# mdolab/adflow

Measured on AMD Instinct MI355X. Metric: Mcells*residual-evals/s, higher is better.
Workload: dtype f64

## Files before the change

### adflow_amd/csrc/api.hip

```cpp
#include <hip/hip_runtime.h>

#include <algorithm>
#include <cmath>
#include <cstdarg>
#include <cstdio>
#include <cstring>
#include <functional>
#include <map>
#include <string>
#include <tuple>
#include <vector>

#include "internal.h"
#include "flow_plan.h"

extern int g_march_kch, g_viscous_tiled, g_inviscid_march, g_roe_march, g_sa_march;
int g_test_fault = 0;
int g_rvec_joint = 1;
int g_pc_fused = 1;
int g_xcd_tiles = 2;

namespace {

std::string g_err;
int g_device = -1;
hipStream_t g_stream = nullptr;
hipStream_t g_streamB = nullptr, g_streamC = nullptr;
hipEvent_t g_evFork = nullptr, g_evB = nullptr, g_evC = nullptr, g_evB1 = nullptr;
hipStream_t g_streamX = nullptr;
hipEvent_t g_evPack = nullptr, g_evComm = nullptr;
int g_overlap = 1;
adflow_opts g_opts;
bool g_have_opts = false;
hipEvent_t g_events[64];
bool g_events_ready = false;
bool g_async = false;

int fail(const char* fmt, ...)
{
    char buf[1024];
    va_list ap;
    va_start(ap, fmt);
    vsnprintf(buf, sizeof buf, fmt, ap);
    va_end(ap);
    g_err = buf;
    return 1;
}

#define HIPCHK(expr)                                                                        \
    do {                                                                                    \
        hipError_t e_ = (expr);                                                             \
        if (e_ != hipSuccess) return fail("%s failed: %s (%s:%d)", #expr, hipGetErrorString(e_), __FILE__, __LINE__); \
    } while (0)

struct DevArr {
    double* base = nullptr;
    int ncomp = 0;
};

struct Block {
    adflow_block_desc d;
    BlkView v;
    long boxsize = 0;
    std::vector<void*> allocs;
// ... 862 lines not shown
        const double* own = which == ADFLOW_ARR_X ? b->d.x : which == ADFLOW_ARR_SI ? b->d.sI : which == ADFLOW_ARR_SJ ? b->d.sJ : b->d.sK;
        const unsigned bit = which == ADFLOW_ARR_X ? 1u : which == ADFLOW_ARR_SI ? 2u : which == ADFLOW_ARR_SJ ? 4u : 8u;
        if (host == own) b->geom_is_host |= bit; else b->geom_is_host &= ~bit;
        b->normals_from_x_ok = b->geom_is_host == 15 && normals_match_nodes(b);
    }
    return sync_and_check();
}

int adflow_gpu_time_step(int level, int onlyRadii)
{
    if (need_ready()) return 1;
    KParams kp = make_kparams(level, 1.0, 0);
    kp.onlyRadii = onlyRadii;
    if (time_step_level(level, kp)) return 1;
    return sync_and_check();
}

int adflow_gpu_initres(int level, int varStart, int varEnd)
{
    if (need_ready()) return 1;
    if (varEnd < varStart) return 0;
    KParams kp = make_kparams(level, 1.0, 0);
    int rc = for_level(level, [&](Block* b) {
        if (varStart < 1 || varEnd > b->v.nw) return fail("initres: variable range %d..%d outside 1..%d", varStart, varEnd, b->v.nw);
        return 0;
    });
    if (rc) return rc;
    LevelTab t;
    if (level_tab(level, &t)) return 1;
    launch_initres_level(t.tab, t.n, t.nx, t.ny, t.nz, kp, varStart - 1, varEnd - 1, g_stream);
    return sync_and_check();
}

static int enqueue_flow_fluxes(int level, const KParams& kp, const struct FlowPlan& P, bool needGrad);
static int source_terms_enqueue(int withBlank);

static int wall_stress_enqueue(int level, const KParams& kp, bool formGrad);

static bool has_wall_subfaces(int level);

static bool level_at_rest(int level)
{
    bool anyMoving = false;
    for_level(level, [&](Block* b) { anyMoving = anyMoving || b->v.sFace || b->v.moving; return 0; });
    return !anyMoving;
}

static void block_face_vectors(Block* b)
{
    if (b->face_vectors_valid) return;
    launch_face_vectors(b->v, g_stream);
    b->face_vectors_valid = true;
}
static int ensure_face_vectors(int level)
{
    return for_level(level, [&](Block* b) { block_face_vectors(b); return 0; });
}

static KParams res_kparams(int level, unsigned flags)
{
    KParams kp = make_kparams(level, 1.0, 0);
    kp.onlyRadii = !(flags & ADFLOW_RES_UPDATE_INTERMED);
    kp.coarseInit = 0;
    if (level == 1 && g_rvec_target) { kp.rvec = g_rvec_target; kp.rvecTurbScale = g_opts.turbResScale; }
    kp.dissApprox = (flags & ADFLOW_RES_DISS_APPROX) ? 1 : 0;
    if (kp.dissApprox && (flags & ADFLOW_RES_UPWIND_FIRST_ORDER)) kp.lumpedDiss = 1;
    return kp;
}

static FlowFacts flow_facts(int level, const KParams& kp, bool viscApprox, bool needGradHbm, bool dual = false,
                            unsigned resFlags = ADFLOW_RES_FLOW)
{
    FlowFacts f = {};
    f.spaceDiscr = kp.spaceDiscr; f.viscous = kp.viscous; f.fineGrid = kp.fineGrid; f.fwMode = kp.fwMode; f.dissApprox = kp.dissApprox;
    f.lumpedDiss = kp.lumpedDiss; f.limiter = kp.limiter; f.coarseInit = kp.coarseInit; f.onlyRadii = kp.onlyRadii;
    f.doScaling = kp.doScaling; f.rvec = kp.rvec != nullptr; f.rFil = kp.rFil; f.adis = kp.adis;
    f.viscApprox = viscApprox; f.needGradHbm = needGradHbm; f.dual = dual;
    f.wantFlow = (resFlags & ADFLOW_RES_FLOW) != 0; f.wantTurb = (resFlags & ADFLOW_RES_TURB) != 0;
    f.atRest = level_at_rest(level);
    f.rans = g_opts.equations == ADFLOW_RANS;
    f.eulerMarch = g_use_march; f.inviscidMarch = g_inviscid_march; f.roeMarch = g_roe_march; f.viscousTiled = g_viscous_tiled;
    f.saMarch = g_sa_march; f.pcFused = g_pc_fused; f.rvecJoint = g_rvec_joint; f.jacSnap = g_jac_snap;
    return f;
}

static int enqueue_flow_residual(int level, const KParams& kp, bool viscApprox = false, bool lowSpeed = true, bool stage0 = true,
                                 bool needGradHbm = false)
{
    const bool wallStress = stage0 && !viscApprox && kp.viscous && level == g_opts.groundLevel && fabs(kp.rFil) >= 1.e-10 &&
                            has_wall_subfaces(level);
    const FlowPlan P = plan_flow(flow_facts(level, kp, viscApprox, needGradHbm));
    if (enqueue_flow_fluxes(level, kp, P, needGradHbm)) return 1;
    if (wallStress)
        if (wall_stress_enqueue(level, kp, P.wallGradOnChip)) return 1;
    if (lowSpeed && level == 1 && source_terms_enqueue(1)) return 1;
    if (lowSpeed && g_opts.lowSpeedPreconditioner) {
        LevelTab t;
        if (level_tab(level, &t)) return 1;
        launch_low_speed_precond_level(t.tab, t.n, t.nx, t.ny, t.nz, kp, g_stream);
    }
    return 0;
}

static int enqueue_flow_fluxes(int level, const KParams& kp, const FlowPlan& P, bool needGrad)
{
    if (kp.spaceDiscr != ADFLOW_DISS_SCALAR && kp.spaceDiscr != ADFLOW_DISS_MATRIX && kp.spaceDiscr != ADFLOW_UPWIND)
        return fail("spaceDiscr=%d not supported (1 scalar, 2 matrix, 9 upwind)", kp.spaceDiscr);
    int nStale = 0, nBlk = 0;
    int rc = for_level(level, [&](Block* b) {
        if (!b->geom_uploaded) return fail("geometry of a level-%d block has not been uploaded", level);
        ++nBlk;
        if (P.needSensor && !b->ss_valid) ++nStale;
        return 0;
    });
    if (rc) return rc;
    if (nStale > 0) {
        if (nStale == nBlk) {
            LevelTab ts;
            if (level_tab(level, &ts)) return 1;
            launch_entropy_level(ts.tab, ts.n, ts.nx, ts.ny, ts.nz, g_stream);
        }
        for_level(level, [&](Block* b) {
            if (nStale != nBlk && !b->ss_valid) launch_entropy(b->v, g_stream);
            b->ss_valid = true;
            return 0;
        });
    }
    LevelTab t;
    if (level_tab(level, &t)) return 1;
    if ((P.needGfTiles && ensure_gf_tiles(level)) || (P.needTiles && ensure_tiles(level))) return 1;
    KParams kv = kp;
    kv.viscFirst = P.viscFirst ? 1 : 0;
    auto inviscid = [&]() -> int {
        switch (P.inviscid) {
        case InviscidK::EulerMarch: launch_euler_march(g_tab[level], g_tiles[level].first, g_tiles[level].second, kv, g_stream); return 0;
        case InviscidK::RoeMarch: return launch_roe_march(g_tab[level], g_tiles[level].first, g_tiles[level].second, kv, g_stream);
        case InviscidK::FaceMarch: return launch_inviscid_march(g_tab[level], g_tiles[level].first, g_tiles[level].second, kv, g_stream);
        case InviscidK::PcMarch: launch_pc_march(g_tab[level], g_tiles[level].first, g_tiles[level].second, kv, g_march_kch, g_stream); return 0;
        case InviscidK::LevelGather: launch_inviscid_level(t.tab, t.n, t.nx, t.ny, t.nz, kv, g_stream); return 0;
        case InviscidK::None: break;
        }
        return 0;
    };
    auto viscous = [&]() -> int {
        switch (P.viscous) {
        case ViscousK::GfMarch: launch_visc_gf(g_tab[level], g_gf_tiles[level].first, g_gf_tiles[level].second, kv, needGrad, g_stream); return 0;
        case ViscousK::ThinLayerMarch: launch_visc_march_approx(g_tab[level], g_tiles[level].first, g_tiles[level].second, kv, g_stream); return 0;
        case ViscousK::GatherExact: return for_level(level, [&](Block* b) { block_face_vectors(b); launch_viscous(b->v, kv, g_stream); return 0; });
        case ViscousK::GatherApprox: return for_level(level, [&](Block* b) { block_face_vectors(b); launch_viscous_approx(b->v, kv, g_stream); return 0; });
        case ViscousK::None: break;
        }
        return 0;
    };
    if (P.inviscid == InviscidK::EulerMarch) return inviscid();
    if (P.inviscid == InviscidK::PcMarch) {
        if (ensure_face_vectors(level)) return 1;
        phase_mark(4);
        if (inviscid()) return 1;
        phase_mark(5);
        return 0;
    }
    if (P.viscFirst) {
        if (ensure_face_vectors(level)) return 1;
        phase_mark(4);
        if (viscous()) return 1;
        phase_mark(5);
        return inviscid();
    }
    if (inviscid()) return 1;
    phase_mark(4);
    if (P.needFaceVectors && ensure_face_vectors(level)) return 1;
    if (P.viscous == ViscousK::GfMarch) phase_mark(5);
    return viscous();
}

int adflow_gpu_residual(int level, int rkStage)
{
    if (need_ready()) return 1;
    double rFil = 1.0;
    int fwMode = 0;
    if (g_opts.smoother == ADFLOW_RUNGE_KUTTA) {
        if (rkStage < 0 || rkStage >= g_opts.nRKStages) return fail("rkStage=%d outside 0..%d", rkStage, g_opts.nRKStages - 1);
        rFil = g_opts.cdisRK[rkStage];
        fwMode = 1;
    }
    KParams kp = make_kparams(level, rFil, fwMode);
    int rc = enqueue_flow_residual(level, kp, false, true, rkStage == 0);
    if (rc) return rc;
    return sync_and_check();
}

static int block_res_enqueue(int level, unsigned flags);
static int apply_bc_enqueue(int level, int secondHalo);
static int apply_turb_bc_enqueue(int level, int secondHalo);
static int apply_turb_and_flow_bc_enqueue(int level, int secondHalo, bool turbBC);
static int turb_bc_treatment_enqueue(int level, const KParams& kp);
static int turb_bc_apply_enqueue(int level, const KParams& kp, int secondHalo);
static int bc_coarse_corrections_enqueue(int coarseLevel, double fact);
static void bc_plan_drop(int level);
static int halo_exchange_enqueue(int level, int varStart, int varEnd, int commPressure, int commVisc, int nLayers);
static int early_pressure_exchange_enqueue(int level);
static int halo_exchange_close(int level, int varStart, int varEnd, int commPressure, int nLayers);
static int comm_exchange_begin(CommPattern* cp, BlkView* tab, unsigned mask, int nvar, bool* remoteOut);
static int comm_exchange_end(CommPattern* cp, BlkView* tab, unsigned mask, bool remote);
static int block_res_split_enqueue(int level, unsigned flags, const KParams& kp, const FlowPlan& P, int lStart, int lEnd, int* taken,
                                   const std::function<int()>& frontBCs);

static int block_res_split_enqueue(int level, unsigned flags, const KParams& kp, const FlowPlan& P, int lStart, int lEnd, int* taken,
                                   const std::function<int()>& frontBCs)
{
    *taken = 0;
    if (!g_split_eval || !g_overlap || g_phase_base > 0 || kp.rvec) return 0;
    const unsigned need = ADFLOW_RES_FLOW | ADFLOW_RES_HALO;
    if ((flags & need) != need || (flags & (ADFLOW_RES_DISS_APPROX | ADFLOW_RES_VISC_APPROX | ADFLOW_RES_UPDATE_INTERMED))) return 0;
    if (P.viscous != ViscousK::GfMarch || !P.viscFirst || (P.inviscid != InviscidK::RoeMarch && P.inviscid != InviscidK::FaceMarch) ||
        P.turb == TurbK::LevelGather || P.needTimeStep || !kp.fineGrid) return 0;
    const bool rans = P.turb == TurbK::SaMarch;
    const bool wall = has_wall_subfaces(level) && level == g_opts.groundLevel;
    if (!g_act.empty()) return 0;
    CommPattern* cp;
    if (build_comm(level, 2, &cp)) return 1;
    const bool messages = !cp->sends.empty() || !cp->recvs.empty();
    if (g_split_eval < 2 && !messages) return 0;
    if (g_bc_callback) return 0;
    unsigned mask; int nvar;
    if (halo_mask(lStart, lEnd, 1, 1, &mask, &nvar)) return 1;
    if (nvar == 0) return 0;
    LevelTab t;
    if (level_tab(level, &t)) return 1;
    int rc = for_level(level, [&](Block* b) {
        if (!b->geom_uploaded) return fail("geometry of a level-%d block has not been uploaded", level);
        if (rans && b->v.nw < 6) return fail("RANS/SA needs nw = 6 (block has %d)", b->v.nw);
        block_face_vectors(b);
        return 0;
    });
    if (rc) return rc;
    if (ensure_tiles(level) || ensure_gf_tiles(level) || (rans && ensure_sa_tiles(level))) return 1;
    *taken = 1;
    KParams kv = kp;
    kv.viscFirst = 1;
    bool forked = false;
    auto run = [&]() -> int {
        HIPCHK(hipEventRecord(g_evFork, g_stream));
        HIPCHK(hipStreamWaitEvent(g_streamB, g_evFork, 0));
        forked = true;
        if (rans) launch_sa_march(t.tab, g_sa_tiles_int[level].first, g_sa_tiles_int[level].second, kp, g_streamB, false);
        launch_visc_gf(g_tab[level], g_gf_tiles_int[level].first, g_gf_tiles_int[level].second, kv, false, g_streamB);
        HIPCHK(hipEventRecord(g_evB1, g_streamB));
        if (frontBCs()) return 1;
        if (g_test_fault & 2) return fail("test_fault: the split evaluation fails behind its fork");
        bool remote = false;
        if (comm_exchange_begin(cp, g_tab[level], mask, nvar, &remote)) return 1;
        if (comm_exchange_end(cp, g_tab[level], mask, remote)) return 1;
        if (halo_exchange_close(level, lStart, lEnd, 1, 2)) return 1;
        HIPCHK(hipEventRecord(g_evC, g_stream));
        HIPCHK(hipStreamWaitEvent(g_streamB, g_evC, 0));
        if (rans) launch_sa_march(t.tab, g_sa_tiles_bnd[level].first, g_sa_tiles_bnd[level].second, kp, g_streamB, false);
        HIPCHK(hipEventRecord(g_evB, g_streamB));
        launch_visc_gf(g_tab[level], g_gf_tiles_bnd[level].first, g_gf_tiles_bnd[level].second, kv, false, g_stream);
        HIPCHK(hipStreamWaitEvent(g_stream, g_evB1, 0));
        if (P.inviscid == InviscidK::RoeMarch ? launch_roe_march(g_tab[level], g_tiles[level].first, g_tiles[level].second, kv, g_stream)
                                              : launch_inviscid_march(g_tab[level], g_tiles[level].first, g_tiles[level].second, kv, g_stream))
            return 1;
        HIPCHK(hipStreamWaitEvent(g_stream, g_evB, 0));
        forked = false;
        return 0;
    };
    if (run()) {
        if (forked && hipEventRecord(g_evB, g_streamB) == hipSuccess) (void)hipStreamWaitEvent(g_stream, g_evB, 0);
        return 1;
    }
    if (wall && wall_stress_enqueue(level, kp, true)) return 1;
    return 0;
}

static int block_res_enqueue(int level, unsigned flags)
{
    if (need_ready()) return 1;
    phase_mark(0);
    KParams kp = res_kparams(level, flags);
    const bool viscApprox = (flags & ADFLOW_RES_VISC_APPROX) != 0;
    const FlowPlan P = plan_flow(flow_facts(level, kp, viscApprox, (flags & ADFLOW_RES_UPDATE_INTERMED) != 0, false, flags));
    int rc = 0;
    bool etotInClosures = false;
    if (flags & ADFLOW_RES_CLOSURES) {
        LevelTab tc;
        if (level_tab(level, &tc)) return 1;
        etotInClosures = (flags & ADFLOW_RES_HALO) && (flags & ADFLOW_RES_FLOW) && g_comm.count(std::make_pair(level, 2)) > 0;
        if (etotInClosures) {
            if (!g_floor_flag_dev) HIPCHK(hipMalloc((void**)&g_floor_flag_dev, sizeof(int)));
            HIPCHK(hipMemsetAsync(g_floor_flag_dev, 0, sizeof(int), g_stream));
        }
        launch_closures_level(tc.tab, tc.n, tc.nx, tc.ny, tc.nz, kp, g_stream, etotInClosures ? g_floor_flag_dev : nullptr);
        rc = for_level(level, [&](Block* b) {
            b->ss_valid = false;
            b->etot_consistent = false;
            return 0;
        });
        if (rc) return rc;
    }
    if (flags & ADFLOW_RES_HALO) {
        auto frontBCs = [&]() -> int {
            if (apply_turb_and_flow_bc_enqueue(level, 1, (flags & ADFLOW_RES_TURB) != 0)) return 1;
            if (g_bc_callback) {
                HIPCHK(hipStreamSynchronize(g_stream));
                g_bc_callback(level, 1);
            }
            return 0;
        };
        int lStart = 1, lEnd = (g_opts.equations == ADFLOW_RANS) ? 6 : 5;
        if ((flags & ADFLOW_RES_FLOW) && !(flags & ADFLOW_RES_TURB)) lEnd = 5;
        if (!(flags & ADFLOW_RES_FLOW) && (flags & ADFLOW_RES_TURB)) lStart = 6;
        if (g_comm.count(std::make_pair(level, 2))) {
            int taken = 0;
            const int flagLevelWas = g_etot_flag_level;
            if (etotInClosures) g_etot_flag_level = level;
            rc = block_res_split_enqueue(level, flags, kp, P, lStart, lEnd, &taken, frontBCs);
            if (!rc && !taken) {
                rc = frontBCs();
                if (!rc) rc = halo_exchange_enqueue(level, lStart, lEnd, 1, 1, 2);
            }
            g_etot_flag_level = flagLevelWas;
            if (rc) return 1;
            if (taken) return 0;
        } else if (frontBCs()) return 1;
    }
    phase_mark(1);
    kp.radiiInMarch = P.radiiInMarch ? 1 : 0;
    if (P.needTimeStep) {
        rc = time_step_level(level, kp);
        if (rc) return rc;
    }
    phase_mark(2);
    if (P.turb != TurbK::None) {
        rc = for_level(level, [&](Block* b) {
            if (b->v.nw < 6) return fail("RANS/SA needs nw = 6 (block has %d)", b->v.nw);
            return 0;
        });
        if (rc) return rc;
        LevelTab t;
        if (level_tab(level, &t)) return 1;
        if (P.turb == TurbK::SaMarch) {
            if (ensure_sa_tiles(level)) return 1;
            if (P.roeWritesTurbRvec) kp.rvecTurbFromDw = 1;
            launch_sa_march(t.tab, g_sa_tiles[level].first, g_sa_tiles[level].second, kp, g_stream, false);
        } else launch_sa_residual_level(t.tab, t.n, t.nx, t.ny, t.nz, kp, g_stream);
    }
    phase_mark(3);
    if (flags & ADFLOW_RES_FLOW) {
        rc = enqueue_flow_residual(level, kp, viscApprox, false, true, (flags & ADFLOW_RES_UPDATE_INTERMED) != 0);
        if (rc) return rc;
    }
    phase_mark(6);
    if (level == 1 && source_terms_enqueue(0)) return 1;
    return 0;
}

int adflow_gpu_actuator_register(int nRegions, const adflow_actuator_region* regions)
// ... 1281 lines not shown
    launch_apply_all_bc(t.tab, pl->d_ent, pl->d_order, pl->flow, kp, secondHalo, g_opts.eulerWallBCTreatment,
                        g_opts.viscWallBCTreatment, g_opts.outflowTreatment, g_opts.hScalingInlet, g_stream);
    return for_level(level, [&](Block* b) {
        if (!b->bc.empty()) b->ss_valid = false;
        return 0;
    });
}

static int ad_apply_bc_enqueue(int level, const KParams& kp, bool turbBC)
{
    BcPlan* pl;
    if (bc_plan(level, &pl)) return 1;
    if (pl->nent == 0) return 0;
    if (pl->anyEulerWall && g_opts.eulerWallBCTreatment == ADFLOW_WALLBC_QUADRATIC)
        return fail("eulerWallBCTreatment=%d: bcEulerWall has no quadratic extrapolation", g_opts.eulerWallBCTreatment);
    LevelTab t;
    if (level_tab(level, &t)) return 1;
    if (turbBC) ad_launch_turb_bc(g_ad_tab, t.n, pl->maxFace, pl->d_ent, pl->d_order, pl->ordinal, kp, 1, g_stream);
    std::vector<BcPhase> flow;
    for (const BcPhase& ph : pl->flow)
        if (ph.kind != BCP_EXTRAP && ph.kind != BCP_SUPERSONIC_INFLOW) flow.push_back(ph);
    ad_launch_apply_all_bc(g_ad_tab, pl->d_ent, pl->d_order, flow, kp, 1, g_opts.eulerWallBCTreatment, g_opts.viscWallBCTreatment,
                           g_opts.outflowTreatment, g_opts.hScalingInlet, g_stream);
    return 0;
}

static bool has_wall_subfaces(int level)
{
    BcPlan* pl;
    if (bc_plan(level, &pl)) return false;
    return pl->wall.count > 0;
}

static int wall_stress_enqueue(int level, const KParams& kp, bool formGrad)
{
    BcPlan* pl;
    if (bc_plan(level, &pl)) return 1;
    if (pl->wall.count == 0) return 0;
    LevelTab t;
    if (level_tab(level, &t)) return 1;
    launch_wall_stress(t.tab, pl->d_ent, pl->d_order, pl->wall, kp, formGrad, g_stream);
    return 0;
}

int adflow_gpu_download_wall_stress(int nn, int level, int sps, int mm, double* tau, double* q)
{
    Block* b = find_block(nn, level, sps);
    if (!b) return fail("block (%d,%d,%d) not registered", nn, level, sps);
    if (mm < 1 || mm > b->nViscBocos || mm > (int)b->bc.size()) return fail("download_wall_stress: subface %d is not a viscous subface of block %d", mm, nn);
    const BcFaceDev& f = b->bc[mm - 1];
    int r[4];
    bc_owned_range(f.faceID, f.icBeg, f.icEnd, f.jcBeg, f.jcEnd, b->v.il, b->v.jl, b->v.kl, r);
    const long no = (long)std::max(0, r[1] - r[0] + 1) * std::max(0, r[3] - r[2] + 1);
    if (no == 0 || !f.tauq) return 0;
    HIPCHK(hipStreamSynchronize(g_stream));
    if (tau) HIPCHK(hipMemcpy(tau, f.tauq, sizeof(double) * 6 * no, hipMemcpyDeviceToHost));
    if (q) HIPCHK(hipMemcpy(q, f.tauq + 6 * no, sizeof(double) * 3 * no, hipMemcpyDeviceToHost));
    return 0;
}

static int bc_coarse_corrections_enqueue(int coarseLevel, double fact)
{
    BcPlan* pl;
    if (bc_plan(coarseLevel, &pl)) return 1;
    if (pl->nent == 0) return 0;
    LevelTab t;
    if (level_tab(coarseLevel, &t)) return 1;
    launch_bc_coarse_corrections(t.tab, pl->d_ent, pl->d_order, pl->ordinal, fact, g_stream);
    return 0;
}

int adflow_gpu_apply_all_bc(int level, int secondHalo)
{
    if (need_ready()) return 1;
// ... 553 lines not shown
        if (!kv.second.h_sendProc.empty() || !kv.second.h_recvProc.empty() || g_comm_self) return false;
    return true;
#endif
}
}

static int mg_cycle_enqueue(const int32_t* cycling, int nSteps);

int adflow_gpu_mg_cycle(const int32_t* cycling, int nSteps)
{
    if (need_ready()) return 1;
    if (!cycling || nSteps < 1) return fail("mg_cycle: empty cycling strategy");
#ifndef HOSTSIM
    if (mg_graph_eligible()) {
        const bool same = (g_mgg.gen == g_state_gen && (int)g_mgg.cyc.size() == nSteps && !memcmp(g_mgg.cyc.data(), cycling, sizeof(int32_t) * nSteps));
        if (!same) {
            mg_graph_drop();
            g_mgg.cyc.assign(cycling, cycling + nSteps);
            g_mgg.gen = g_state_gen;
        }
        if (g_mgg.exec && block_flags() == g_mgg.pre) {
            HIPCHK(hipGraphLaunch(g_mgg.exec, g_stream));
            set_block_flags(g_mgg.post);
            return sync_and_check();
        }
        if (g_mgg.exec) {
            g_mgg.seen = 0;
        } else if (g_mgg.seen >= 1) {
            HIPCHK(hipStreamSynchronize(g_stream));
            g_mgg.pre = block_flags();
            if (hipStreamBeginCapture(g_stream, hipStreamCaptureModeThreadLocal) == hipSuccess) {
                const bool was = g_async;
                g_async = true;
                const int rc = mg_cycle_enqueue(cycling, nSteps);
                g_async = was;
                hipGraph_t gr = nullptr;
                const hipError_t e1 = hipStreamEndCapture(g_stream, &gr);
                if (rc == 0 && e1 == hipSuccess && gr && !(g_test_fault & 1) && hipGraphInstantiate(&g_mgg.exec, gr, nullptr, nullptr, 0) == hipSuccess) {
                    g_mgg.graph = gr;
                    g_mgg.post = block_flags();
                    HIPCHK(hipGraphLaunch(g_mgg.exec, g_stream));
                    return sync_and_check();
                }
                if (gr) (void)hipGraphDestroy(gr);
                (void)hipGetLastError();
                g_mgg.exec = nullptr;
                g_mgg.failed = true;
                set_block_flags(g_mgg.pre);
            } else {
                (void)hipGetLastError();
                g_mgg.failed = true;
            }
        }
        ++g_mgg.seen;
    }
#endif
    const bool was_async = g_async;
    g_async = true;
    const int rc = mg_cycle_enqueue(cycling, nSteps);
    g_async = was_async;
    if (rc) return rc;
    return sync_and_check();
}

static int mg_cycle_enqueue(const int32_t* cycling, int nSteps)
{
    int level = g_opts.groundLevel;
// ... 536 lines not shown
        std::vector<int4> h((size_t)tt.second);
        if (tt.second > 0) HIPCHK(hipMemcpy(h.data(), tt.first, sizeof(int4) * h.size(), hipMemcpyDeviceToHost));
        for (const int4& t : h)
            if (t.x >= 0) out[1] += 4.0 * (t.w - t.z + 3);
    }
    for (auto& kv : g_blocks) {
        if (std::get<0>(kv.first) != level || std::get<1>(kv.first) != 1) continue;
        const BlkView& v = kv.second->v;
        int ntx, nty, ntz;
        euler_march_tiles(v, &ntx, &nty, &ntz);
        out[2] += 4.0 * ntx * nty * (v.nz + ntz);
    }
    return 0;
}

int adflow_gpu_sync(void)
{
    if (g_device < 0) return fail("adflow_gpu_init has not been called");
    HIPCHK(hipGetLastError());
    HIPCHK(hipStreamSynchronize(g_stream));
    return 0;
}

int adflow_gpu_set_tuning(const char* key, int value)
{
    ++g_state_gen;
    if (!key) return fail("null tuning key");
    if (!strcmp(key, "euler_march")) { g_use_march = (value != 0); return 0; }
    if (!strcmp(key, "viscous_tiled")) { g_viscous_tiled = value; return 0; }
    if (!strcmp(key, "inviscid_march")) { g_inviscid_march = value; return 0; }
    if (!strcmp(key, "roe_march")) { g_roe_march = value; return 0; }
    if (!strcmp(key, "sa_march")) { g_sa_march = value; return 0; }
    if (!strcmp(key, "overlap")) { g_overlap = value; return 0; }
    if (!strcmp(key, "max_grid_z")) { g_max_grid_z = (value > 0) ? value : 65535; return 0; }
    if (!strcmp(key, "metric_from_x")) { g_metric_from_x = value; return 0; }
    if (!strcmp(key, "xcd_tiles")) {
        g_xcd_tiles = value;
        if (g_stream) (void)hipStreamSynchronize(g_stream);
        mg_graph_drop();
        for (auto& kv : g_tiles) (void)hipFree(kv.second.first);
        g_tiles.clear();
        return 0;
    }
    if (!strcmp(key, "phase_events")) {
        if (value != 0 && (value < 8 || value > 56)) return fail("phase_events: first slot must be 8..56 (or 0 = off)");
        g_phase_base = value;
        return 0;
    }
    if (!strcmp(key, "march_kch")) {
        if (value < 4) return fail("march_kch must be >= 4");
        g_march_kch = value;
        if (g_stream) (void)hipStreamSynchronize(g_stream);
        mg_graph_drop();
        for (auto* mp : {&g_tiles, &g_gf_tiles, &g_gf_tiles_int, &g_gf_tiles_bnd, &g_sa_tiles, &g_sa_tiles_int, &g_sa_tiles_bnd}) {
            for (auto& kv : *mp) (void)hipFree(kv.second.first);
            mp->clear();
        }
        return 0;
    }
    if (!strcmp(key, "split_eval")) { g_split_eval = value; return 0; }
    if (!strcmp(key, "test_fault")) { g_test_fault = value; g_mgg.failed = false; mg_graph_drop(); return 0; }
    if (!strcmp(key, "ad_cache")) { g_ad_cache = value; if (!value) { if (g_stream) (void)hipStreamSynchronize(g_stream); ad_drop(); } return 0; }
    if (!strcmp(key, "rvec_joint")) { g_rvec_joint = value; return 0; }
    if (!strcmp(key, "jac_snap")) { g_jac_snap = value; return 0; }
    if (!strcmp(key, "pc_fused")) { g_pc_fused = value; mg_graph_drop(); return 0; }
    if (!strcmp(key, "mg_graph")) { g_mg_graph = value; g_mgg.failed = false; mg_graph_drop(); return 0; }
// ... 65 lines not shown
```

### adflow_amd/csrc/internal.h

```cpp
#pragma once
#include <hip/hip_runtime.h>
#include <stdint.h>
#include "../../include/adflow_gpu.h"

#define ADF_PAD0 14

#ifdef HOSTSIM
#define GPTR(T) T*
#else
#define GPTR(T) T __attribute__((address_space(1)))*
#endif

__device__ __forceinline__ double ldg(GPTR(const double) base, unsigned byteoff)
{
    return *(GPTR(const double))((GPTR(const char))base + byteoff);
}
__device__ __forceinline__ void stg(GPTR(double) base, unsigned byteoff, double v)
{
    *(GPTR(double))((GPTR(char))base + byteoff) = v;
}

#ifndef ADF_NR
#define ADF_NR 1
#endif
// ... 347 lines not shown
void launch_source_terms(const BlkView* tab, const int* blk, const long* off, int n, const double Ffact[3], double Qfact, int withBlank,
                         hipStream_t s);
void launch_low_speed_precond_level(const BlkView* tab, int nslots, int maxnx, int maxny, int maxnz, const KParams& kp, hipStream_t s);
void launch_stage_update_level(const BlkView* tab, int nslots, int maxnx, int maxny, int maxnz, const KParams& kp, double scale,
                               int fromWn, hipStream_t s);
void launch_res_averaging_level(const BlkView* tab, int nslots, int maxnx, int maxny, int maxnz, const KParams& kp, hipStream_t s,
                                double scaleDtl = 0.0);
void launch_dadi_level(const BlkView* tab, int nslots, int nx, int ny, int nz, const KParams& kp, hipStream_t s, bool withUpdate = false);
void launch_halo_copy(const BlkView* tab, const int* donorBlk, const long* donorOff, const int* haloBlk, const long* haloOff,
                      int n, unsigned mask, hipStream_t s);
void launch_periodic(const BlkView* tab, const int* blk, const long* off, int n, const double rotMatrix[9], const double rotCenter[3],
                     const double translation[3], int coor, hipStream_t s);
void launch_halo_pack(const BlkView* tab, const int* blk, const long* off, int n, unsigned mask, double* buf, hipStream_t s);
void launch_halo_unpack(const BlkView* tab, const int* blk, const long* off, int n, unsigned mask, const double* buf,
                        hipStream_t s);
int launch_inviscid_march(const BlkView* tab, const int4* tiles, int ntiles, const KParams& kp, hipStream_t s);
int inviscid_march_enabled();
int launch_roe_march(const BlkView* tab, const int4* tiles, int ntiles, const KParams& kp, hipStream_t s);
void launch_pc_march(const BlkView* tab, const int4* tiles, int ntiles, const KParams& kp, int kch, hipStream_t s);
bool roe_march_takes(int limiter);
void launch_euler_march(const BlkView* tab, const int4* tiles, int ntiles, const KParams& kp, hipStream_t s);
void euler_march_tiles(const BlkView& b, int* ntx, int* nty, int* ntz);
void launch_restrict_level(const BlkView* ctab, const BlkView* ftab, int nslots, int nx, int ny, int nz, const KParams& kp, hipStream_t s);
void launch_store_entry_state_level(const BlkView* ctab, int nslots, int nx, int ny, int nz, hipStream_t s);
void launch_forcing_level(const BlkView* ctab, int nslots, int nx, int ny, int nz, double fcoll, hipStream_t s);
void launch_corrections_level(const BlkView* ctab, int nslots, int nx, int ny, int nz, hipStream_t s);
void launch_prolong_update_level(const BlkView* ftab, const BlkView* ctab, int nslots, int nx, int ny, int nz, const KParams& kp,
                                 hipStream_t s);
void launch_set_w(const BlkView& b, const double* vec, double turbFloor, hipStream_t s);
void launch_get_r(const BlkView& b, double* vec, double turbScale, double* sums, hipStream_t s);
void launch_closures(const BlkView& b, const KParams& kp, hipStream_t s);
void launch_closures_level(const BlkView* tab, int nslots, int maxnx, int maxny, int maxnz, const KParams& kp, hipStream_t s,
                           int* floored = nullptr);
void launch_set_w_closures_level(const BlkView* tab, int nslots, int maxnx, int maxny, int maxnz, const double* vec, double turbFloor,
                                 const KParams& kp, int* floored, hipStream_t s);
void launch_set_w_level(const BlkView* tab, int nslots, int maxnx, int maxny, int maxnz, const double* vec, double turbFloor, hipStream_t s);
void launch_get_r_level(const BlkView* tab, int nslots, int maxnx, int maxny, int maxnz, double* vec, double turbScale, double* sums, hipStream_t s);
void launch_entropy_level(const BlkView* tab, int nslots, int maxnx, int maxny, int maxnz, hipStream_t s);
void launch_etot_owned_level(const BlkView* tab, int nslots, int maxnx, int maxny, int maxnz, double gammaConstant, hipStream_t s,
                             const int* onlyIf = nullptr);
void launch_initres_level(const BlkView* tab, int nslots, int maxnx, int maxny, int maxnz, const KParams& kp, int l0, int l1, hipStream_t s);
void launch_res_norms(const BlkView& b, int nvar, double* out, hipStream_t s);
#include <vector>
void launch_apply_all_bc(const BlkView* tab, const BcEntry* ent, const int* order, const std::vector<BcPhase>& flow,
                         const KParams& kp, int second, int eulerWallTreatment, int viscWallTreatment, int outflowTreatment, int hScalingInlet,
                         hipStream_t s);
void launch_turb_bc_treatment(const BlkView* tab, int nslots, long maxFace, const BcEntry* ent, const int* order,
                              const std::vector<BcPhase>& ordinal, const KParams& kp, hipStream_t s);
void launch_apply_turb_bc(const BlkView* tab, const BcEntry* ent, const int* order, const std::vector<BcPhase>& ordinal,
                          const KParams& kp, int second, hipStream_t s);
void launch_bc_coarse_corrections(const BlkView* tab, const BcEntry* ent, const int* order, const std::vector<BcPhase>& ordinal,
                                  double fact, hipStream_t s);
void launch_corner_row_halos_level(const BlkView* tab, int nslots, const KParams& kp, hipStream_t s);
void launch_volume_metric(const BlkView& b, int rightHanded, hipStream_t s);
void launch_boundary_normals(const BlkView& b, const BcFaceDev* faces, int nBocos, hipStream_t s);
void launch_wall_distance(const BlkView& b, const int* ind, const double* uv, const double* xSurf, hipStream_t s);

void ad_launch_from_real(const double* src, void* dst, long n, hipStream_t s);
void ad_launch_value(const void* src, double* dst, long n, int deriv, hipStream_t s);
void ad_launch_snap(const BlkView& b, const void* dwd, double* snap, const JacSpec& J, double turbResScale, hipStream_t s);
void ad_launch_closures_halo(const BlkView& adv, const KParams& kp, hipStream_t s);
void ad_launch_apply_all_bc(const BlkView* tab, const BcEntry* ent, const int* order, const std::vector<BcPhase>& flow, const KParams& kp,
                            int second, int eulerWallTreatment, int viscWallTreatment, int outflowTreatment, int hScalingInlet, hipStream_t s);
void ad_launch_turb_bc(const BlkView* tab, int nslots, long maxFace, const BcEntry* ent, const int* order, const std::vector<BcPhase>& ordinal,
                       const KParams& kp, int second, hipStream_t s);
void ad_launch_time_step_level(const BlkView* tab, int n, int nx, int ny, int nz, const KParams& kp, hipStream_t s);
// ... 15 lines not shown
```

### adflow_amd/csrc/kernels_nk.hip

```cpp
#include <algorithm>

#include "internal.h"

#define NK_BX 64
#define NK_BY 4

__device__ __forceinline__ void set_w_body(const BlkView& b, int kz, const double* __restrict__ vec, double turbFloor)
{
    const int i = blockIdx.x * NK_BX + threadIdx.x + 2;
    const int j = blockIdx.y * NK_BY + threadIdx.y + 2;
    const int k = kz + 2;
    if (i > b.il || j > b.jl || k > b.kl) return;
    const long c = b.idx(i, j, k);
    const long m = (((long)(k - 2) * b.ny + (j - 2)) * b.nx + (i - 2)) * b.nw;
    for (int l = 0; l < 5; ++l) b.w[c + l * b.nbox] = vec[m + l];
    if (b.nw > 5) b.w[c + 5 * b.nbox] = fmax(turbFloor, vec[m + 5]);
}

__global__ __launch_bounds__(NK_BX* NK_BY) void k_set_w(BlkView b, const double* __restrict__ vec, double turbFloor)
{
    set_w_body(b, (int)blockIdx.z, vec, turbFloor);
}

__global__ __launch_bounds__(NK_BX* NK_BY) void k_set_w_level(const BlkView* __restrict__ tab, int nzb, const double* __restrict__ vec,
// ... 88 lines not shown
    }
    if (kp.viscous) {
        const double muSuth = kp.muSuthDim / kp.muRef, TSuth = kp.TSuthDim / kp.TRef, SSuth = kp.SSuthDim / kp.TRef;
        const double T = p / (kp.RGas * rho);
        const double tt = T / TSuth;
        const double rlv = muSuth * ((TSuth + SSuth) / (T + SSuth)) * (tt * sqrt(tt));
        b.rlv[c] = rlv;
        if (kp.eddyModel && kp.updateEddy) {
            const double cv13 = kp.sa_cv1 * kp.sa_cv1 * kp.sa_cv1;
            const double rnuSA = b.w[c + 5 * nb] * rho;
            const double chi = rnuSA / rlv;
            const double chi3 = chi * chi * chi;
            b.rev[c] = chi3 / (chi3 + cv13) * rnuSA;
        }
    }
}

__global__ __launch_bounds__(NK_BX* NK_BY) void k_closures(BlkView b, KParams kp) { closures_body(b, (int)blockIdx.z, kp); }

__global__ __launch_bounds__(NK_BX* NK_BY) void k_set_w_closures_level(const BlkView* __restrict__ tab, int nzb, const double* __restrict__ vec,
                                                                       double turbFloor, KParams kp, int* __restrict__ floored)
{
    const BlkView& b = tab[blockIdx.z / nzb + 1];
    set_w_body(b, (int)(blockIdx.z % nzb), vec + b.vecOff, turbFloor);
    closures_body<true>(b, (int)(blockIdx.z % nzb), kp, floored);
}

template <bool ETOT>
__global__ __launch_bounds__(NK_BX* NK_BY) void k_closures_level(const BlkView* __restrict__ tab, int nzb, KParams kp, int* __restrict__ floored)
{
    closures_body<ETOT>(tab[blockIdx.z / nzb + 1], (int)(blockIdx.z % nzb), kp, floored);
}

static dim3 nk_grid(const BlkView& b) { return dim3((b.nx + NK_BX - 1) / NK_BX, (b.ny + NK_BY - 1) / NK_BY, b.nz); }
static dim3 nk_level_grid(int nslots, int maxnx, int maxny, int maxnz)
{
    return dim3((maxnx + NK_BX - 1) / NK_BX, (maxny + NK_BY - 1) / NK_BY, maxnz * nslots);
}

void launch_closures_level(const BlkView* tab, int nslots, int maxnx, int maxny, int maxnz, const KParams& kp, hipStream_t s, int* floored)
{
    LEVEL_SPLIT(nslots, maxnz + 4, launch_closures_level(tab + s0_, n_, maxnx, maxny, maxnz, kp, s, floored));
    if (nslots <= 0) return;
    if (floored)
        hipLaunchKernelGGL(k_closures_level<true>, nk_level_grid(nslots, maxnx, maxny, maxnz), dim3(NK_BX, NK_BY, 1), 0, s, tab, maxnz, kp, floored);
    else
        hipLaunchKernelGGL(k_closures_level<false>, nk_level_grid(nslots, maxnx, maxny, maxnz), dim3(NK_BX, NK_BY, 1), 0, s, tab, maxnz, kp,
                           (int*)nullptr);
}
void launch_set_w_closures_level(const BlkView* tab, int nslots, int maxnx, int maxny, int maxnz, const double* vec, double turbFloor,
                                 const KParams& kp, int* floored, hipStream_t s)
{
    LEVEL_SPLIT(nslots, maxnz + 4, launch_set_w_closures_level(tab + s0_, n_, maxnx, maxny, maxnz, vec, turbFloor, kp, floored, s));
    if (nslots <= 0) return;
    hipLaunchKernelGGL(k_set_w_closures_level, nk_level_grid(nslots, maxnx, maxny, maxnz), dim3(NK_BX, NK_BY, 1), 0, s, tab, maxnz, vec, turbFloor,
                       kp, floored);
}
void launch_set_w_level(const BlkView* tab, int nslots, int maxnx, int maxny, int maxnz, const double* vec, double turbFloor, hipStream_t s)
{
    LEVEL_SPLIT(nslots, maxnz + 4, launch_set_w_level(tab + s0_, n_, maxnx, maxny, maxnz, vec, turbFloor, s));
    if (nslots <= 0) return;
    hipLaunchKernelGGL(k_set_w_level, nk_level_grid(nslots, maxnx, maxny, maxnz), dim3(NK_BX, NK_BY, 1), 0, s, tab, maxnz, vec, turbFloor);
}
void launch_get_r_level(const BlkView* tab, int nslots, int maxnx, int maxny, int maxnz, double* vec, double turbScale, double* sums, hipStream_t s)
{
    LEVEL_SPLIT(nslots, maxnz + 4, launch_get_r_level(tab + s0_, n_, maxnx, maxny, maxnz, vec, turbScale, sums, s));
    if (nslots <= 0) return;
    hipLaunchKernelGGL(k_get_r_level, nk_level_grid(nslots, maxnx, maxny, maxnz), dim3(NK_BX, NK_BY, 1), 0, s, tab, maxnz, vec, turbScale, sums);
}

void launch_set_w(const BlkView& b, const double* vec, double turbFloor, hipStream_t s)
{
    hipLaunchKernelGGL(k_set_w, nk_grid(b), dim3(NK_BX, NK_BY, 1), 0, s, b, vec, turbFloor);
}

void launch_get_r(const BlkView& b, double* vec, double turbScale, double* sums, hipStream_t s)
{
    hipLaunchKernelGGL(k_get_r, nk_grid(b), dim3(NK_BX, NK_BY, 1), 0, s, b, vec, turbScale, sums);
}

void launch_closures(const BlkView& b, const KParams& kp, hipStream_t s)
{
// ... 3 lines not shown
```

Baseline: 4874.

## Split closures into shell and bulk, overlap bulk and wall stress on side stream

The closures kernel is split into a shell launch covering the outer two layers of each block and a bulk launch covering the interior. The shell runs first, so boundary conditions and halo exchange can start while the interior closures run on a second stream and join before the fluxes. The wall-stress kernel is likewise moved to the side stream after the viscous-first pass so it can overlap the inviscid fluxes. This adds launches, events and more complex indexing in exchange for hiding closure and wall-stress work behind the front BCs and comms. Side-stream use is turned off during graph capture and when callbacks are active.

```diff
diff --git a/adflow_amd/csrc/api.hip b/adflow_amd/csrc/api.hip
--- a/adflow_amd/csrc/api.hip
+++ b/adflow_amd/csrc/api.hip
@@ -30,6 +30,8 @@
 hipStream_t g_streamX = nullptr;
 hipEvent_t g_evPack = nullptr, g_evComm = nullptr;
 int g_overlap = 1;
+int g_closures_split = 1;
+bool g_capturing = false;
 adflow_opts g_opts;
 bool g_have_opts = false;
 hipEvent_t g_events[64];
@@ -958,10 +960,12 @@
     return sync_and_check();
 }
 
-static int enqueue_flow_fluxes(int level, const KParams& kp, const struct FlowPlan& P, bool needGrad);
+static int enqueue_flow_fluxes(int level, const KParams& kp, const struct FlowPlan& P, bool needGrad,
+                               const std::function<int()>* afterViscousFirst = nullptr);
 static int source_terms_enqueue(int withBlank);
 
-static int wall_stress_enqueue(int level, const KParams& kp, bool formGrad);
+static int wall_stress_enqueue(int level, const KParams& kp, bool formGrad, hipStream_t s = g_stream);
+static bool side_queue_usable() { return g_overlap && g_phase_base == 0 && !g_bc_callback && !g_capturing; }
 
 static bool has_wall_subfaces(int level);
 
@@ -1016,9 +1020,23 @@
     const bool wallStress = stage0 && !viscApprox && kp.viscous && level == g_opts.groundLevel && fabs(kp.rFil) >= 1.e-10 &&
                             has_wall_subfaces(level);
     const FlowPlan P = plan_flow(flow_facts(level, kp, viscApprox, needGradHbm));
-    if (enqueue_flow_fluxes(level, kp, P, needGradHbm)) return 1;
-    if (wallStress)
-        if (wall_stress_enqueue(level, kp, P.wallGradOnChip)) return 1;
+    const bool wallBeside = wallStress && P.viscFirst && side_queue_usable();
+    bool forkMarked = false;
+    const std::function<int()> markFork = [&]() -> int {
+        HIPCHK(hipEventRecord(g_evFork, g_stream));
+        forkMarked = true;
+        return 0;
+    };
+    if (enqueue_flow_fluxes(level, kp, P, needGradHbm, wallBeside ? &markFork : nullptr)) return 1;
+    if (wallStress) {
+        if (forkMarked) {
+            HIPCHK(hipStreamWaitEvent(g_streamB, g_evFork, 0));
+            const int rc = wall_stress_enqueue(level, kp, P.wallGradOnChip, g_streamB);
+            if (hipEventRecord(g_evB, g_streamB) != hipSuccess || hipStreamWaitEvent(g_stream, g_evB, 0) != hipSuccess)
+                return fail("the side queue of the wall stress could not be joined");
+            if (rc) return rc;
+        } else if (wall_stress_enqueue(level, kp, P.wallGradOnChip)) return 1;
+    }
     if (lowSpeed && level == 1 && source_terms_enqueue(1)) return 1;
     if (lowSpeed && g_opts.lowSpeedPreconditioner) {
         LevelTab t;
@@ -1028,7 +1046,7 @@
     return 0;
 }
 
-static int enqueue_flow_fluxes(int level, const KParams& kp, const FlowPlan& P, bool needGrad)
+static int enqueue_flow_fluxes(int level, const KParams& kp, const FlowPlan& P, bool needGrad, const std::function<int()>* afterViscousFirst)
 {
     if (kp.spaceDiscr != ADFLOW_DISS_SCALAR && kp.spaceDiscr != ADFLOW_DISS_MATRIX && kp.spaceDiscr != ADFLOW_UPWIND)
         return fail("spaceDiscr=%d not supported (1 scalar, 2 matrix, 9 upwind)", kp.spaceDiscr);
@@ -1091,6 +1109,7 @@
         phase_mark(4);
         if (viscous()) return 1;
         phase_mark(5);
+        if (afterViscousFirst && (*afterViscousFirst)()) return 1;
         return inviscid();
     }
     if (inviscid()) return 1;
@@ -1129,29 +1148,42 @@
 static int halo_exchange_close(int level, int varStart, int varEnd, int commPressure, int nLayers);
 static int comm_exchange_begin(CommPattern* cp, BlkView* tab, unsigned mask, int nvar, bool* remoteOut);
 static int comm_exchange_end(CommPattern* cp, BlkView* tab, unsigned mask, bool remote);
+static int comm_exchange_enqueue(CommPattern* cp, BlkView* tab, unsigned mask, int nvar);
 static int block_res_split_enqueue(int level, unsigned flags, const KParams& kp, const FlowPlan& P, int lStart, int lEnd, int* taken,
                                    const std::function<int()>& frontBCs);
+static bool split_eval_applies(int level, unsigned flags, const KParams& kp, const FlowPlan& P, int lStart, int lEnd, int* err);
+
+static bool split_eval_applies(int level, unsigned flags, const KParams& kp, const FlowPlan& P, int lStart, int lEnd, int* err)
+{
+    *err = 0;
+    if (!g_split_eval || !g_overlap || g_phase_base > 0 || kp.rvec) return false;
+    const unsigned need = ADFLOW_RES_FLOW | ADFLOW_RES_HALO;
+    if ((flags & need) != need || (flags & (ADFLOW_RES_DISS_APPROX | ADFLOW_RES_VISC_APPROX | ADFLOW_RES_UPDATE_INTERMED))) return false;
+    if (P.viscous != ViscousK::GfMarch || !P.viscFirst || (P.inviscid != InviscidK::RoeMarch && P.inviscid != InviscidK::FaceMarch) ||
+        P.turb == TurbK::LevelGather || P.needTimeStep || !kp.fineGrid) return false;
+    if (!g_act.empty()) return false;
+    CommPattern* cp;
+    if (build_comm(level, 2, &cp)) { *err = 1; return false; }
+    const bool messages = !cp->sends.empty() || !cp->recvs.empty();
+    if (g_split_eval < 2 && !messages) return false;
+    if (g_bc_callback) return false;
+    unsigned mask; int nvar;
+    if (halo_mask(lStart, lEnd, 1, 1, &mask, &nvar)) { *err = 1; return false; }
+    return nvar > 0;
+}
 
 static int block_res_split_enqueue(int level, unsigned flags, const KParams& kp, const FlowPlan& P, int lStart, int lEnd, int* taken,
                                    const std::function<int()>& frontBCs)
 {
     *taken = 0;
-    if (!g_split_eval || !g_overlap || g_phase_base > 0 || kp.rvec) return 0;
-    const unsigned need = ADFLOW_RES_FLOW | ADFLOW_RES_HALO;
-    if ((flags & need) != need || (flags & (ADFLOW_RES_DISS_APPROX | ADFLOW_RES_VISC_APPROX | ADFLOW_RES_UPDATE_INTERMED))) return 0;
-    if (P.viscous != ViscousK::GfMarch || !P.viscFirst || (P.inviscid != InviscidK::RoeMarch && P.inviscid != InviscidK::FaceMarch) ||
-        P.turb == TurbK::LevelGather || P.needTimeStep || !kp.fineGrid) return 0;
+    int err = 0;
+    if (!split_eval_applies(level, flags, kp, P, lStart, lEnd, &err)) return err;
     const bool rans = P.turb == TurbK::SaMarch;
     const bool wall = has_wall_subfaces(level) && level == g_opts.groundLevel;
-    if (!g_act.empty()) return 0;
     CommPattern* cp;
     if (build_comm(level, 2, &cp)) return 1;
-    const bool messages = !cp->sends.empty() || !cp->recvs.empty();
-    if (g_split_eval < 2 && !messages) return 0;
-    if (g_bc_callback) return 0;
     unsigned mask; int nvar;
     if (halo_mask(lStart, lEnd, 1, 1, &mask, &nvar)) return 1;
-    if (nvar == 0) return 0;
     LevelTab t;
     if (level_tab(level, &t)) return 1;
     int rc = for_level(level, [&](Block* b) {
@@ -1209,15 +1241,37 @@
     const FlowPlan P = plan_flow(flow_facts(level, kp, viscApprox, (flags & ADFLOW_RES_UPDATE_INTERMED) != 0, false, flags));
     int rc = 0;
     bool etotInClosures = false;
+    bool bulkPending = false;
+    LevelTab tc;
+    int lStart = 1, lEnd = (g_opts.equations == ADFLOW_RANS) ? 6 : 5;
+    if ((flags & ADFLOW_RES_FLOW) && !(flags & ADFLOW_RES_TURB)) lEnd = 5;
+    if (!(flags & ADFLOW_RES_FLOW) && (flags & ADFLOW_RES_TURB)) lStart = 6;
+    auto bulkClosures = [&](hipStream_t s) -> int {
+        if (!bulkPending) return 0;
+        bulkPending = false;
+        launch_closures_bulk_level(tc.tab, tc.n, tc.nx, tc.ny, tc.nz, kp, s, etotInClosures ? g_floor_flag_dev : nullptr);
+        return 0;
+    };
     if (flags & ADFLOW_RES_CLOSURES) {
-        LevelTab tc;
         if (level_tab(level, &tc)) return 1;
         etotInClosures = (flags & ADFLOW_RES_HALO) && (flags & ADFLOW_RES_FLOW) && g_comm.count(std::make_pair(level, 2)) > 0;
         if (etotInClosures) {
             if (!g_floor_flag_dev) HIPCHK(hipMalloc((void**)&g_floor_flag_dev, sizeof(int)));
             HIPCHK(hipMemsetAsync(g_floor_flag_dev, 0, sizeof(int), g_stream));
         }
-        launch_closures_level(tc.tab, tc.n, tc.nx, tc.ny, tc.nz, kp, g_stream, etotInClosures ? g_floor_flag_dev : nullptr);
+        int* const floorFlag = etotInClosures ? g_floor_flag_dev : nullptr;
+        int err = 0;
+        const bool splitEval = etotInClosures && split_eval_applies(level, flags, kp, P, lStart, lEnd, &err);
+        if (err) return 1;
+        if (g_closures_split >= 2) {
+            if (g_closures_split == 2) launch_closures_shell_level(tc.tab, tc.n, tc.nx, tc.ny, tc.nz, kp, g_stream, floorFlag);
+            else launch_closures_bulk_level(tc.tab, tc.n, tc.nx, tc.ny, tc.nz, kp, g_stream, floorFlag);
+        } else if (g_closures_split == 1 && (flags & ADFLOW_RES_HALO) && kp.fineGrid && !splitEval &&
+                   std::min(tc.nx, std::min(tc.ny, tc.nz)) > 2 * CLOSURE_SHELL) {
+            launch_closures_shell_level(tc.tab, tc.n, tc.nx, tc.ny, tc.nz, kp, g_stream, floorFlag);
+            bulkPending = true;
+        } else
+            launch_closures_level(tc.tab, tc.n, tc.nx, tc.ny, tc.nz, kp, g_stream, floorFlag);
         rc = for_level(level, [&](Block* b) {
             b->ss_valid = false;
             b->etot_consistent = false;
@@ -1234,22 +1288,48 @@
             }
             return 0;
         };
-        int lStart = 1, lEnd = (g_opts.equations == ADFLOW_RANS) ? 6 : 5;
-        if ((flags & ADFLOW_RES_FLOW) && !(flags & ADFLOW_RES_TURB)) lEnd = 5;
-        if (!(flags & ADFLOW_RES_FLOW) && (flags & ADFLOW_RES_TURB)) lStart = 6;
+        auto frontWithBulk = [&](bool exchange) -> int {
+            bool forked = false;
+            auto run = [&]() -> int {
+                if (bulkPending && side_queue_usable()) {
+                    HIPCHK(hipEventRecord(g_evFork, g_stream));
+                    HIPCHK(hipStreamWaitEvent(g_streamB, g_evFork, 0));
+                    forked = true;
+                    if (bulkClosures(g_streamB)) return 1;
+                    HIPCHK(hipEventRecord(g_evB, g_streamB));
+                }
+                if (frontBCs()) return 1;
+                if (g_test_fault & 4) return fail("test_fault: the boundary front fails behind its fork");
+                unsigned mask = 0; int nvar = 0;
+                if (exchange) {
+                    CommPattern* cp;
+                    if (build_comm(level, 2, &cp)) return 1;
+                    if (halo_mask(lStart, lEnd, 1, 1, &mask, &nvar)) return 1;
+                    if (nvar > 0 && comm_exchange_enqueue(cp, g_tab[level], mask, nvar)) return 1;
+                }
+                if (bulkClosures(g_stream)) return 1;
+                if (forked) {
+                    HIPCHK(hipStreamWaitEvent(g_stream, g_evB, 0));
+                    forked = false;
+                }
+                return (exchange && nvar > 0) ? halo_exchange_close(level, lStart, lEnd, 1, 2) : 0;
+            };
+            if (run()) {
+                if (forked && hipEventRecord(g_evB, g_streamB) == hipSuccess) (void)hipStreamWaitEvent(g_stream, g_evB, 0);
+                return 1;
+            }
+            return 0;
+        };
         if (g_comm.count(std::make_pair(level, 2))) {
             int taken = 0;
             const int flagLevelWas = g_etot_flag_level;
             if (etotInClosures) g_etot_flag_level = level;
             rc = block_res_split_enqueue(level, flags, kp, P, lStart, lEnd, &taken, frontBCs);
-            if (!rc && !taken) {
-                rc = frontBCs();
-                if (!rc) rc = halo_exchange_enqueue(level, lStart, lEnd, 1, 1, 2);
-            }
+            if (!rc && !taken) rc = frontWithBulk(true);
             g_etot_flag_level = flagLevelWas;
             if (rc) return 1;
             if (taken) return 0;
-        } else if (frontBCs()) return 1;
+        } else if (frontWithBulk(false)) return 1;
     }
     phase_mark(1);
     kp.radiiInMarch = P.radiiInMarch ? 1 : 0;
@@ -2597,14 +2677,14 @@
     return pl->wall.count > 0;
 }
 
-static int wall_stress_enqueue(int level, const KParams& kp, bool formGrad)
+static int wall_stress_enqueue(int level, const KParams& kp, bool formGrad, hipStream_t s)
 {
     BcPlan* pl;
     if (bc_plan(level, &pl)) return 1;
     if (pl->wall.count == 0) return 0;
     LevelTab t;
     if (level_tab(level, &t)) return 1;
-    launch_wall_stress(t.tab, pl->d_ent, pl->d_order, pl->wall, kp, formGrad, g_stream);
+    launch_wall_stress(t.tab, pl->d_ent, pl->d_order, pl->wall, kp, formGrad, s);
     return 0;
 }
 
@@ -3224,7 +3304,9 @@
             if (hipStreamBeginCapture(g_stream, hipStreamCaptureModeThreadLocal) == hipSuccess) {
                 const bool was = g_async;
                 g_async = true;
+                g_capturing = true;
                 const int rc = mg_cycle_enqueue(cycling, nSteps);
+                g_capturing = false;
                 g_async = was;
                 hipGraph_t gr = nullptr;
                 const hipError_t e1 = hipStreamEndCapture(g_stream, &gr);
@@ -3827,6 +3909,20 @@
     if (!strcmp(key, "roe_march")) { g_roe_march = value; return 0; }
     if (!strcmp(key, "sa_march")) { g_sa_march = value; return 0; }
     if (!strcmp(key, "overlap")) { g_overlap = value; return 0; }
+    if (!strcmp(key, "closures_split")) { g_closures_split = value; return 0; }
+    if (!strcmp(key, "side_priority")) {
+#ifndef HOSTSIM
+        if (!g_streamB) return fail("side_priority: adflow_gpu_init has not been called");
+        if (g_stream) (void)hipStreamSynchronize(g_stream);
+        (void)hipStreamSynchronize(g_streamB);
+        int least = 0, greatest = 0;
+        HIPCHK(hipDeviceGetStreamPriorityRange(&least, &greatest));
+        HIPCHK(hipStreamDestroy(g_streamB));
+        g_streamB = nullptr;
+        HIPCHK(hipStreamCreateWithPriority(&g_streamB, hipStreamNonBlocking, value ? least : 0));
+#endif
+        return 0;
+    }
     if (!strcmp(key, "max_grid_z")) { g_max_grid_z = (value > 0) ? value : 65535; return 0; }
     if (!strcmp(key, "metric_from_x")) { g_metric_from_x = value; return 0; }
     if (!strcmp(key, "xcd_tiles")) {
diff --git a/adflow_amd/csrc/internal.h b/adflow_amd/csrc/internal.h
--- a/adflow_amd/csrc/internal.h
+++ b/adflow_amd/csrc/internal.h
@@ -403,6 +403,11 @@
 void launch_closures(const BlkView& b, const KParams& kp, hipStream_t s);
 void launch_closures_level(const BlkView* tab, int nslots, int maxnx, int maxny, int maxnz, const KParams& kp, hipStream_t s,
                            int* floored = nullptr);
+#define CLOSURE_SHELL 2
+void launch_closures_shell_level(const BlkView* tab, int nslots, int maxnx, int maxny, int maxnz, const KParams& kp, hipStream_t s,
+                                 int* floored = nullptr);
+void launch_closures_bulk_level(const BlkView* tab, int nslots, int maxnx, int maxny, int maxnz, const KParams& kp, hipStream_t s,
+                                int* floored = nullptr);
 void launch_set_w_closures_level(const BlkView* tab, int nslots, int maxnx, int maxny, int maxnz, const double* vec, double turbFloor,
                                  const KParams& kp, int* floored, hipStream_t s);
 void launch_set_w_level(const BlkView* tab, int nslots, int maxnx, int maxny, int maxnz, const double* vec, double turbFloor, hipStream_t s);
diff --git a/adflow_amd/csrc/kernels_nk.hip b/adflow_amd/csrc/kernels_nk.hip
--- a/adflow_amd/csrc/kernels_nk.hip
+++ b/adflow_amd/csrc/kernels_nk.hip
@@ -144,6 +144,58 @@
     closures_body<ETOT>(tab[blockIdx.z / nzb + 1], (int)(blockIdx.z % nzb), kp, floored);
 }
 
+__device__ __forceinline__ int shell_layer(int q, int n) { return (q < CLOSURE_SHELL || n <= 2 * CLOSURE_SHELL) ? q : n - 2 * CLOSURE_SHELL + q; }
+__host__ __device__ inline int shell_count(int n) { return n < 2 * CLOSURE_SHELL ? n : 2 * CLOSURE_SHELL; }
+__host__ __device__ inline void shell_groups(int nx, int ny, int nz, int g[3])
+{
+    const int nxc = (nx + NK_BX - 1) / NK_BX;
+    const int nkS = shell_count(nz), njS = shell_count(ny), niS = shell_count(nx);
+    g[0] = nxc * ((nkS * ny + NK_BY - 1) / NK_BY);
+    g[1] = nxc * (((nz - nkS) * njS + NK_BY - 1) / NK_BY);
+    g[2] = (int)(((long)(nz - nkS) * (ny - njS) * niS + NK_BX * NK_BY - 1) / (NK_BX * NK_BY));
+}
+
+template <bool ETOT>
+__global__ __launch_bounds__(NK_BX* NK_BY) void k_closures_shell_level(const BlkView* __restrict__ tab, KParams kp, int* __restrict__ floored)
+{
+    const BlkView& b = tab[blockIdx.y + 1];
+    const int nx = b.nx, ny = b.ny, nz = b.nz;
+    if (nx == 0) return;
+    int ng[3];
+    shell_groups(nx, ny, nz, ng);
+    const int nxc = (nx + NK_BX - 1) / NK_BX;
+    int g = (int)blockIdx.x;
+    if (g < ng[0] + ng[1]) {
+        const bool famA = g < ng[0];
+        if (!famA) g -= ng[0];
+        const int njS = shell_count(ny);
+        const int ii = (g % nxc) * NK_BX + (int)threadIdx.x, r = (g / nxc) * NK_BY + (int)threadIdx.y;
+        const int rows = famA ? shell_count(nz) * ny : (nz - shell_count(nz)) * njS;
+        if (ii >= nx || r >= rows) return;
+        const int jj = famA ? r % ny : shell_layer(r % njS, ny);
+        const int kk = famA ? shell_layer(r / ny, nz) : CLOSURE_SHELL + r / njS;
+        closures_cell<ETOT>(b, ii + 2, jj + 2, kk + 2, kp, floored);
+        return;
+    }
+    g -= ng[0] + ng[1];
+    const int niS = shell_count(nx), njI = ny - shell_count(ny), nkI = nz - shell_count(nz);
+    const long t = (long)g * (NK_BX * NK_BY) + threadIdx.y * NK_BX + threadIdx.x;
+    if (t >= (long)nkI * njI * niS) return;
+    const int ii = shell_layer((int)(t % niS), nx), jj = CLOSURE_SHELL + (int)((t / niS) % njI), kk = CLOSURE_SHELL + (int)(t / ((long)niS * njI));
+    closures_cell<ETOT>(b, ii + 2, jj + 2, kk + 2, kp, floored);
+}
+
+template <bool ETOT>
+__global__ __launch_bounds__(NK_BX* NK_BY) void k_closures_bulk_level(const BlkView* __restrict__ tab, int nzb, KParams kp, int* __restrict__ floored)
+{
+    const BlkView& b = tab[blockIdx.z / nzb + 1];
+    const int ii = blockIdx.x * NK_BX + threadIdx.x;
+    const int jj = blockIdx.y * NK_BY + threadIdx.y + CLOSURE_SHELL;
+    const int kk = (int)(blockIdx.z % nzb) + CLOSURE_SHELL;
+    if (ii < CLOSURE_SHELL || ii >= b.nx - CLOSURE_SHELL || jj >= b.ny - CLOSURE_SHELL || kk >= b.nz - CLOSURE_SHELL) return;
+    closures_cell<ETOT>(b, ii + 2, jj + 2, kk + 2, kp, floored);
+}
+
 static dim3 nk_grid(const BlkView& b) { return dim3((b.nx + NK_BX - 1) / NK_BX, (b.ny + NK_BY - 1) / NK_BY, b.nz); }
 static dim3 nk_level_grid(int nslots, int maxnx, int maxny, int maxnz)
 {
@@ -160,6 +212,26 @@
         hipLaunchKernelGGL(k_closures_level<false>, nk_level_grid(nslots, maxnx, maxny, maxnz), dim3(NK_BX, NK_BY, 1), 0, s, tab, maxnz, kp,
                            (int*)nullptr);
 }
+void launch_closures_shell_level(const BlkView* tab, int nslots, int maxnx, int maxny, int maxnz, const KParams& kp, hipStream_t s, int* floored)
+{
+    LEVEL_SPLIT(nslots, 1, launch_closures_shell_level(tab + s0_, n_, maxnx, maxny, maxnz, kp, s, floored));
+    if (nslots <= 0) return;
+    int ng[3];
+    shell_groups(maxnx, maxny, maxnz, ng);
+    const dim3 grid(ng[0] + ng[1] + ng[2], nslots, 1);
+    if (grid.x == 0) return;
+    if (floored) hipLaunchKernelGGL(k_closures_shell_level<true>, grid, dim3(NK_BX, NK_BY, 1), 0, s, tab, kp, floored);
+    else hipLaunchKernelGGL(k_closures_shell_level<false>, grid, dim3(NK_BX, NK_BY, 1), 0, s, tab, kp, (int*)nullptr);
+}
+void launch_closures_bulk_level(const BlkView* tab, int nslots, int maxnx, int maxny, int maxnz, const KParams& kp, hipStream_t s, int* floored)
+{
+    LEVEL_SPLIT(nslots, maxnz + 4, launch_closures_bulk_level(tab + s0_, n_, maxnx, maxny, maxnz, kp, s, floored));
+    const int bx = maxnx - 2 * CLOSURE_SHELL, by = maxny - 2 * CLOSURE_SHELL, bz = maxnz - 2 * CLOSURE_SHELL;
+    if (nslots <= 0 || bx <= 0 || by <= 0 || bz <= 0) return;
+    const dim3 grid((maxnx + NK_BX - 1) / NK_BX, (by + NK_BY - 1) / NK_BY, bz * nslots);
+    if (floored) hipLaunchKernelGGL(k_closures_bulk_level<true>, grid, dim3(NK_BX, NK_BY, 1), 0, s, tab, bz, kp, floored);
+    else hipLaunchKernelGGL(k_closures_bulk_level<false>, grid, dim3(NK_BX, NK_BY, 1), 0, s, tab, bz, kp, (int*)nullptr);
+}
 void launch_set_w_closures_level(const BlkView* tab, int nslots, int maxnx, int maxny, int maxnz, const double* vec, double turbFloor,
                                  const KParams& kp, int* floored, hipStream_t s)
 {
```

New measurement: 4801. -1.5%, worse.
